# ruotianluo/ImageCaptioning.pytorch

Measured on NVIDIA H100. Metric: captions/sec at beam=5 seq_len=20, higher is better.
Workload: dtype f32 (fp32-grade: split-fp16 x3 tensor-core passes, fp32 accumulate)

## Files before the change

imagecaptioning.pytorch_b200/csrc/gemm_tc.cu:

```cuda
#include <cstdlib>

#include "common.cuh"
#include "ptx.cuh"

namespace capb200 {

namespace {

constexpr int BM = 128;
constexpr int BK = 64;
constexpr int kConsumers = 2;
constexpr int kThreads = 128 * (1 + kConsumers);

struct TcParams {
    CUtensorMap a_hi[kMaxSeg];
    CUtensorMap a_lo[kMaxSeg];
    CUtensorMap w_hi[kMaxSeg];
    CUtensorMap w_lo[kMaxSeg];
    int kblocks[kMaxSeg];
    int nseg;
    int M, N;
    float* C;
    long ldc;
    __half* C_hi;
    __half* C_lo;
    long ldcs;
    const float* bias;
    const float* row_bias;
    long ld_row_bias;
    int rows_per_group;
    int relu;
    const float* residual;
    long ld_res;
    int tiles_m, tiles_n;
    int lstm, H;
    const float* c_prev;
    long ld_cprev;
    const int* src_row;
    float* c_out;
    long ld_cout;
    const float* gather_bias;
    long ld_gb;
    const int* gather_idx;
    float* h_f;
    __half* h_hi;
    __half* h_lo;
    long ld_h;
    unsigned long long* trace;
};

__device__ __forceinline__ unsigned long long gtimer() {
    unsigned long long t;
    asm volatile("mov.u64 %0, %%globaltimer;" : "=l"(t));
    return t;
}
#define CAPB_TRACE(slot) do { if (TRACE && p.trace != nullptr) p.trace[(long)blockIdx.x * 16 + (slot)] = gtimer(); } while (0)

template <int BN, int PASSES>
struct TcCfg {
    static constexpr int kPlanes = (PASSES == 3) ? 2 : 1;
    static constexpr uint32_t kABytes = BM * BK * 2;
    static constexpr uint32_t kWBytes = BN * BK * 2;
    static constexpr uint32_t kStageBytes = kPlanes * (kABytes + kWBytes);
    static constexpr uint32_t kRingBudget = 227 * 1024 - 1024  - 256 ;
    static constexpr int kStages = kRingBudget / kStageBytes >= 8 ? 8 : kRingBudget / kStageBytes;
    static constexpr uint32_t kSmemBytes = kStages * kStageBytes + 1024  + 256 ;
    static_assert(BN == 64 || BN == 128 || BN == 160, "wgmma wrappers exist for N = 64, 128 and 160");
    static_assert(kWBytes % 1024 == 0, "operand tiles must keep the 1024-byte swizzle-atom alignment");
    static_assert(kStages >= 2, "need at least a double buffer");
    static_assert(kSmemBytes <= 227 * 1024, "shared memory of one H100 block");
};

template <int BN>
__device__ __forceinline__ void wgmma_f16(float* acc, uint64_t da, uint64_t db, int scale_d) {
    if (BN == 160) ptx::wgmma_f16_n160(acc, da, db, scale_d);
    else if (BN == 128) ptx::wgmma_f16_n128(acc, da, db, scale_d);
    else ptx::wgmma_f16_n64(acc, da, db, scale_d);
}

enum EpiKind : int {
    kEpiStore = 0,
    kEpiPlanes = 1,
    kEpiLstm = 2,
};

template <int BN>
__device__ __forceinline__ void epi_adds(const TcParams& p, float* acc, int r0, int c0) {
    const int ncol = p.N - c0;
    const int lim[2] = {r0 < p.M ? ncol : 0, r0 + 8 < p.M ? ncol : 0};
    if (p.bias != nullptr) {
        const float* b = p.bias + c0;
#pragma unroll
        for (int j = 0; j < BN / 8; ++j) {
#pragma unroll
            for (int e = 0; e < 2; ++e) {
                if (8 * j + e < ncol) {
                    const float x = __ldg(b + 8 * j + e);
                    acc[4 * j + e] += x;
                    acc[4 * j + 2 + e] += x;
                }
            }
        }
    }
    const float* tab[3][2];
#pragma unroll
    for (int h = 0; h < 2; ++h) {
        const int row = lim[h] > 0 ? r0 + 8 * h : 0;
        tab[0][h] = p.row_bias != nullptr ? p.row_bias + (long)(row / p.rows_per_group) * p.ld_row_bias + c0 : nullptr;
        tab[1][h] = p.gather_bias != nullptr ? p.gather_bias + (long)(lim[h] > 0 ? p.gather_idx[row] : 0) * p.ld_gb + c0 : nullptr;
        tab[2][h] = p.residual != nullptr ? p.residual + (long)row * p.ld_res + c0 : nullptr;
    }
#pragma unroll 1
    for (int t = 0; t < 3; ++t) {
        const float* const t0 = t == 0 ? tab[0][0] : t == 1 ? tab[1][0] : tab[2][0];
        const float* const t1 = t == 0 ? tab[0][1] : t == 1 ? tab[1][1] : tab[2][1];
        if (t0 == nullptr) continue;
#pragma unroll
        for (int j = 0; j < BN / 8; ++j) {
#pragma unroll
            for (int e = 0; e < 4; ++e) {
                const int k = 8 * j + (e & 1);
                if (k < lim[e >> 1]) acc[4 * j + e] += (e >> 1 ? t1 : t0)[k];
            }
        }
    }
    if (p.relu) {
#pragma unroll
        for (int i = 0; i < BN / 2; ++i) acc[i] = fmaxf(acc[i], 0.0f);
    }
}

template <int BN, bool TRACE>
__device__ __forceinline__ void epi_lstm(const TcParams& p, float* acc, int r0, int c0, int lane, int slot) {
    constexpr int kRuns = BN / 32;
    const bool odd = lane & 1;
    const bool upper = lane & 2;
    const int row = r0 + (odd ? 8 : 0);
    const int u0 = ((c0 - 2 * (lane & 3)) >> 2) + (upper ? 4 : 0);
    const bool row_ok = row < p.M;
    const bool full = u0 + 8 * (kRuns - 1) + 4 <= p.H;
    int src = row;
    if (p.src_row != nullptr && row_ok) src = p.src_row[row];
    const float* cprev = (row_ok && src >= 0 && p.c_prev != nullptr) ? p.c_prev + (long)src * p.ld_cprev + u0 : nullptr;
    float cp[BN / 8];
    if (cprev != nullptr && full && (reinterpret_cast<uintptr_t>(cprev) & 15) == 0) {
#pragma unroll
        for (int k = 0; k < kRuns; ++k) {
            const float4 v = *reinterpret_cast<const float4*>(cprev + 8 * k);
            cp[4 * k] = v.x; cp[4 * k + 1] = v.y; cp[4 * k + 2] = v.z; cp[4 * k + 3] = v.w;
        }
    } else {
#pragma unroll
        for (int i = 0; i < BN / 8; ++i) {
            const int du = 8 * (i / 4) + i % 4;
            cp[i] = (cprev != nullptr && u0 + du < p.H) ? cprev[du] : 0.0f;
        }
    }
    if (TRACE && slot >= 0) {
        float s = 0.0f;
#pragma unroll
        for (int i = 0; i < BN / 8; ++i) s += cp[i];
        asm volatile("" ::"f"(s));
        CAPB_TRACE(slot);
    }
    __syncwarp();
#pragma unroll
    for (int j = 0; j < BN / 8; ++j) {
        float* v = acc + 4 * j;
        const float s0 = __shfl_xor_sync(0xffffffffu, odd ? v[0] : v[2], 1);
        const float s1 = __shfl_xor_sync(0xffffffffu, odd ? v[1] : v[3], 1);
        const float gi = odd ? s0 : v[0], gf = odd ? s1 : v[1], gg = odd ? v[2] : s0, go = odd ? v[3] : s1;
        v[0] = gi; v[1] = gf; v[2] = gg; v[3] = go;
    }
#pragma unroll
    for (int k = 0; k < kRuns; ++k) {
#pragma unroll
        for (int t = 0; t < 2; ++t) {
            float* x = acc + 4 * (4 * k + t);
            float* y = acc + 4 * (4 * k + 2 + t);
#pragma unroll
            for (int g = 0; g < 4; ++g) {
                const float keep = upper ? y[g] : x[g];
                const float recv = __shfl_xor_sync(0xffffffffu, upper ? x[g] : y[g], 2);
                x[g] = upper ? recv : keep;
                y[g] = upper ? keep : recv;
            }
        }
    }
    float cn[BN / 8], hn[BN / 8];
#pragma unroll
    for (int i = 0; i < BN / 8; ++i) {
        const int k = i / 4, o = i % 4;
        const float* g = acc + 4 * (4 * k + (o >> 1) + 2 * (o & 1));
        cn[i] = fast_sigmoid(g[1]) * cp[i] + fast_sigmoid(g[0]) * fast_tanh(g[2]);
        hn[i] = fast_sigmoid(g[3]) * fast_tanh(cn[i]);
    }
    if (TRACE && slot >= 0) {
        float s = 0.0f;
#pragma unroll
        for (int i = 0; i < BN / 8; ++i) s += hn[i];
        asm volatile("" ::"f"(s));
        CAPB_TRACE(slot + 1);
    }
    if (row_ok) {
        float* const c_out = p.c_out + (long)row * p.ld_cout + u0;
        float* const h_f = p.h_f + (long)row * p.ld_h + u0;
        __half* const h_hi = p.h_hi + (long)row * p.ld_h + u0;
        __half* const h_lo = p.h_lo + (long)row * p.ld_h + u0;
        const bool planes = p.h_hi != nullptr;
        const uintptr_t a16 = reinterpret_cast<uintptr_t>(c_out) | reinterpret_cast<uintptr_t>(h_f);
        const uintptr_t a8 = planes ? reinterpret_cast<uintptr_t>(h_hi) | reinterpret_cast<uintptr_t>(h_lo) : 0;
        if (full && (a16 & 15) == 0 && (a8 & 7) == 0) {
#pragma unroll
            for (int k = 0; k < kRuns; ++k) {
                const float* c = cn + 4 * k;
                const float* h = hn + 4 * k;
                *reinterpret_cast<float4*>(c_out + 8 * k) = make_float4(c[0], c[1], c[2], c[3]);
                *reinterpret_cast<float4*>(h_f + 8 * k) = make_float4(h[0], h[1], h[2], h[3]);
                if (planes) {
                    __half hh[4], hl[4];
#pragma unroll
                    for (int o = 0; o < 4; ++o) split_f32(h[o], hh[o], hl[o]);
                    const __half2 hi01 = __halves2half2(hh[0], hh[1]), hi23 = __halves2half2(hh[2], hh[3]);
                    const __half2 lo01 = __halves2half2(hl[0], hl[1]), lo23 = __halves2half2(hl[2], hl[3]);
                    *reinterpret_cast<uint2*>(h_hi + 8 * k) = make_uint2(*reinterpret_cast<const uint32_t*>(&hi01), *reinterpret_cast<const uint32_t*>(&hi23));
                    *reinterpret_cast<uint2*>(h_lo + 8 * k) = make_uint2(*reinterpret_cast<const uint32_t*>(&lo01), *reinterpret_cast<const uint32_t*>(&lo23));
                }
            }
        } else {
#pragma unroll
            for (int i = 0; i < BN / 8; ++i) {
                const int du = 8 * (i / 4) + i % 4;
                if (u0 + du < p.H) {
                    c_out[du] = cn[i];
                    h_f[du] = hn[i];
                    if (planes) {
                        __half hh, hl;
                        split_f32(hn[i], hh, hl);
                        h_hi[du] = hh;
                        h_lo[du] = hl;
                    }
                }
            }
        }
    }
    if (TRACE && slot >= 0) CAPB_TRACE(slot + 2);
}

template <int BN, bool PLANES>
__device__ __forceinline__ void epi_store(const TcParams& p, const float* acc, int r0, int c0) {
    const int ncol = p.N - c0;
#pragma unroll
    for (int h = 0; h < 2; ++h) {
        const int row = r0 + 8 * h;
        if (row >= p.M) continue;
        if (p.C != nullptr) {
            float* const dst = p.C + (long)row * p.ldc + c0;
            if (ncol >= BN && (reinterpret_cast<uintptr_t>(dst) & 7) == 0) {
#pragma unroll
                for (int j = 0; j < BN / 8; ++j) *reinterpret_cast<float2*>(dst + 8 * j) = make_float2(acc[4 * j + 2 * h], acc[4 * j + 2 * h + 1]);
            } else {
#pragma unroll
                for (int j = 0; j < BN / 8; ++j) {
                    if (8 * j < ncol) dst[8 * j] = acc[4 * j + 2 * h];
                    if (8 * j + 1 < ncol) dst[8 * j + 1] = acc[4 * j + 2 * h + 1];
                }
            }
        }
        if (PLANES) {
            __half* const dh = p.C_hi + (long)row * p.ldcs + c0;
            __half* const dl = p.C_lo + (long)row * p.ldcs + c0;
            if (ncol >= BN && ((reinterpret_cast<uintptr_t>(dh) | reinterpret_cast<uintptr_t>(dl)) & 3) == 0) {
#pragma unroll
                for (int j = 0; j < BN / 8; ++j) {
                    __half h0, l0, h1, l1;
                    split_f32(acc[4 * j + 2 * h], h0, l0);
                    split_f32(acc[4 * j + 2 * h + 1], h1, l1);
                    *reinterpret_cast<__half2*>(dh + 8 * j) = __halves2half2(h0, h1);
                    *reinterpret_cast<__half2*>(dl + 8 * j) = __halves2half2(l0, l1);
                }
            } else {
#pragma unroll
                for (int j = 0; j < BN / 8; ++j) {
#pragma unroll
                    for (int e = 0; e < 2; ++e) {
                        __half hi, lo;
                        split_f32(acc[4 * j + 2 * h + e], hi, lo);
                        if (8 * j + e < ncol) { dh[8 * j + e] = hi; dl[8 * j + e] = lo; }
                    }
                }
            }
        }
    }
}

template <int BN, int EPI, bool TRACE>
__device__ __forceinline__ void epilogue_tile(const TcParams& p, float* acc, int m0, int n0, int tid, int slot) {
    const int warp = tid >> 5, lane = tid & 31;
    const int r0 = m0 + warp * 16 + (lane >> 2);
    const int c0 = n0 + 2 * (lane & 3);
    epi_adds<BN>(p, acc, r0, c0);
    if (EPI == kEpiLstm) epi_lstm<BN, TRACE>(p, acc, r0, c0, lane, slot);
    else epi_store<BN, EPI == kEpiPlanes>(p, acc, r0, c0);
}

template <int BN, int PASSES, int EPI, bool TRACE = false>
__global__ void __launch_bounds__(kThreads, 1) gemm_tc_kernel(const __grid_constant__ TcParams p) {
    using Cfg = TcCfg<BN, PASSES>;
    extern __shared__ uint8_t smem_raw[];
    uint8_t* smem = reinterpret_cast<uint8_t*>((reinterpret_cast<uintptr_t>(smem_raw) + 1023) & ~uintptr_t(1023));
    uint64_t* full_bar = reinterpret_cast<uint64_t*>(smem + Cfg::kStages * Cfg::kStageBytes);
    uint64_t* empty_bar = full_bar + Cfg::kStages;
    uint64_t* turn_bar = empty_bar + Cfg::kStages;

    const int wg = threadIdx.x >> 7;
    const int n_tiles = p.tiles_m * p.tiles_n;

    if (threadIdx.x == 0) {
        for (int s = 0; s < p.nseg; ++s) {
            ptx::prefetch_tmap(&p.a_hi[s]);
            ptx::prefetch_tmap(&p.w_hi[s]);
            if (PASSES == 3) {
                ptx::prefetch_tmap(&p.a_lo[s]);
                ptx::prefetch_tmap(&p.w_lo[s]);
            }
        }
        for (int i = 0; i < Cfg::kStages; ++i) {
            ptx::mbar_init(&full_bar[i], 1);
            ptx::mbar_init(&empty_bar[i], 1);
        }
        for (int c = 0; c < kConsumers; ++c) ptx::mbar_init(&turn_bar[c], 1);
        ptx::fence_mbar_init();
    }
    __syncthreads();
    if (threadIdx.x == 0) CAPB_TRACE(0);

    if (wg == 0) {
        ptx::setmaxnreg_dec<40>();
        if (threadIdx.x == 0) {
            int stage = 0;
            uint32_t phase = 0;
            for (int t = blockIdx.x; t < n_tiles; t += gridDim.x) {
                const int m0 = (t % p.tiles_m) * BM;
                const int n0 = (t / p.tiles_m) * BN;
                for (int s = 0; s < p.nseg; ++s) {
                    for (int kb = 0; kb < p.kblocks[s]; ++kb) {
                        ptx::mbar_wait(&empty_bar[stage], phase ^ 1);
                        uint8_t* st = smem + stage * Cfg::kStageBytes;
                        uint8_t* a_hi = st;
                        uint8_t* a_lo = st + Cfg::kABytes;
                        uint8_t* w_hi = st + Cfg::kABytes * Cfg::kPlanes;
                        uint8_t* w_lo = st + Cfg::kABytes * 2 + Cfg::kWBytes;
                        ptx::mbar_arrive_expect_tx(&full_bar[stage], Cfg::kStageBytes);
                        ptx::tma_load_2d(a_hi, &p.a_hi[s], &full_bar[stage], kb * BK, m0);
                        ptx::tma_load_2d(w_hi, &p.w_hi[s], &full_bar[stage], kb * BK, n0);
                        if (PASSES == 3) {
                            ptx::tma_load_2d(a_lo, &p.a_lo[s], &full_bar[stage], kb * BK, m0);
                            ptx::tma_load_2d(w_lo, &p.w_lo[s], &full_bar[stage], kb * BK, n0);
                        }
                        if (++stage == Cfg::kStages) { stage = 0; phase ^= 1; }
                    }
                }
            }
        }
    } else {
        ptx::setmaxnreg_inc<232>();
        const int cw = wg - 1;
        const int tid = threadIdx.x & 127;
        constexpr uint32_t kHalf = 64 * 128;
        int kb_tile = 0;
        for (int s = 0; s < p.nseg; ++s) kb_tile += p.kblocks[s];
        int mine = 0;
        for (int it = cw, t = blockIdx.x + cw * gridDim.x; t < n_tiles; it += 2, t += 2 * gridDim.x, ++mine) {
            const int m0 = (t % p.tiles_m) * BM;
            const int n0 = (t / p.tiles_m) * BN;
            if (it > 0) ptx::mbar_wait(&turn_bar[cw], (cw == 1 ? mine : mine - 1) & 1);
            if (TRACE && it == 1 && tid == 0) CAPB_TRACE(4);
            const long g0 = (long)it * kb_tile;
            int stage = (int)(g0 % Cfg::kStages);
            uint32_t phase = (uint32_t)(g0 / Cfg::kStages) & 1;
            float acc0[BN / 2], acc1[BN / 2];
#pragma unroll
            for (int i = 0; i < BN / 2; ++i) { acc0[i] = 0.0f; acc1[i] = 0.0f; }
            for (int s = 0; s < p.nseg; ++s) {
                for (int kb = 0; kb < p.kblocks[s]; ++kb) {
                    ptx::mbar_wait(&full_bar[stage], phase);
                    if (TRACE && it == 0 && s == 0 && kb == 0 && tid == 0) CAPB_TRACE(1);
                    const uint32_t st = ptx::smem_u32(smem + stage * Cfg::kStageBytes);
                    const uint32_t a_hi = st;
                    const uint32_t a_lo = st + Cfg::kABytes;
                    const uint32_t w_hi = st + Cfg::kABytes * Cfg::kPlanes;
                    const uint32_t w_lo = st + Cfg::kABytes * 2 + Cfg::kWBytes;
#pragma unroll
                    for (int i = 0; i < BN / 2; ++i) { ptx::reg_fence(acc0[i]); ptx::reg_fence(acc1[i]); }
                    ptx::wgmma_fence();
#pragma unroll
                    for (int k = 0; k < BK / 16; ++k) {
                        const uint32_t koff = k * 32;
                        const uint64_t dwh = ptx::make_smem_desc_sw128(w_hi + koff);
                        if (PASSES == 3) {
                            const uint64_t dwl = ptx::make_smem_desc_sw128(w_lo + koff);
                            wgmma_f16<BN>(acc0, ptx::make_smem_desc_sw128(a_hi + koff), dwl, 1);
                            wgmma_f16<BN>(acc1, ptx::make_smem_desc_sw128(a_hi + kHalf + koff), dwl, 1);
                            wgmma_f16<BN>(acc0, ptx::make_smem_desc_sw128(a_lo + koff), dwh, 1);
                            wgmma_f16<BN>(acc1, ptx::make_smem_desc_sw128(a_lo + kHalf + koff), dwh, 1);
                            wgmma_f16<BN>(acc0, ptx::make_smem_desc_sw128(a_hi + koff), dwh, 1);
                            wgmma_f16<BN>(acc1, ptx::make_smem_desc_sw128(a_hi + kHalf + koff), dwh, 1);
                        } else {
                            wgmma_f16<BN>(acc0, ptx::make_smem_desc_sw128(a_hi + koff), dwh, 1);
                            wgmma_f16<BN>(acc1, ptx::make_smem_desc_sw128(a_hi + kHalf + koff), dwh, 1);
                        }
                    }
                    ptx::wgmma_commit();
                    ptx::wgmma_wait<0>();
#pragma unroll
                    for (int i = 0; i < BN / 2; ++i) { ptx::reg_fence(acc0[i]); ptx::reg_fence(acc1[i]); }
                    if (tid == 0) ptx::mbar_arrive(&empty_bar[stage]);
                    if (++stage == Cfg::kStages) { stage = 0; phase ^= 1; }
                }
            }
            if (tid == 0) ptx::mbar_arrive(&turn_bar[cw ^ 1]);
            if (TRACE && it < 2 && tid == 0) CAPB_TRACE(2 + it);
#pragma unroll 1
            for (int h = 0; h < 2; ++h) {
                const int slot = (TRACE && it < 2 && h == 0 && tid == 0) ? 9 + 3 * it : -1;
                epilogue_tile<BN, EPI, TRACE>(p, acc0, m0 + 64 * h, n0, tid, slot);
#pragma unroll
                for (int i = 0; i < BN / 2; ++i) acc0[i] = acc1[i];
            }
            if (TRACE && it < 2 && tid == 0) CAPB_TRACE(6 + it);
        }
    }
    __syncthreads();
    if (threadIdx.x == 0) CAPB_TRACE(8);
}

typedef CUresult (*EncodeTiledFn)(CUtensorMap*, CUtensorMapDataType, cuuint32_t, void*, const cuuint64_t*, const cuuint64_t*,
                                  const cuuint32_t*, const cuuint32_t*, CUtensorMapInterleave, CUtensorMapSwizzle,
                                  CUtensorMapL2promotion, CUtensorMapFloatOOBfill);

EncodeTiledFn get_encode_fn() {
    static EncodeTiledFn fn = nullptr;
    if (fn == nullptr) {
        void* sym = nullptr;
        cudaDriverEntryPointQueryResult qres;
        if (cudaGetDriverEntryPoint("cuTensorMapEncodeTiled", &sym, cudaEnableDefault, &qres) != cudaSuccess || sym == nullptr) {
            return nullptr;
        }
        fn = reinterpret_cast<EncodeTiledFn>(sym);
    }
    return fn;
}

bool encode_plane(CUtensorMap* map, const __half* base, long rows, long K, long pitch, int box_rows, std::string* err) {
    EncodeTiledFn fn = get_encode_fn();
    if (fn == nullptr) { *err = "cuTensorMapEncodeTiled entry point not available"; return false; }
    cuuint64_t gdim[2] = {static_cast<cuuint64_t>(K), static_cast<cuuint64_t>(rows)};
    cuuint64_t gstride[1] = {static_cast<cuuint64_t>(pitch) * 2};
    cuuint32_t box[2] = {static_cast<cuuint32_t>(BK), static_cast<cuuint32_t>(box_rows)};
    cuuint32_t estr[2] = {1, 1};
    CUresult r = fn(map, CU_TENSOR_MAP_DATA_TYPE_FLOAT16, 2, const_cast<__half*>(base), gdim, gstride, box, estr,
                    CU_TENSOR_MAP_INTERLEAVE_NONE, CU_TENSOR_MAP_SWIZZLE_128B, CU_TENSOR_MAP_L2_PROMOTION_L2_256B,
                    CU_TENSOR_MAP_FLOAT_OOB_FILL_NONE);
    if (r != CUDA_SUCCESS) { *err = "cuTensorMapEncodeTiled failed with CUresult " + std::to_string((int)r); return false; }
    return true;
}

template <int BN, int PASSES, int EPI, bool TRACE = false>
int launch_cfg(const TcParams& prm, cudaStream_t stream) {
    using Cfg = TcCfg<BN, PASSES>;
    static std::atomic<unsigned long long> attr_set{0};
    if (first_use_on_device(attr_set)) {
        CAPB_CHECK_CUDA(cudaFuncSetAttribute(gemm_tc_kernel<BN, PASSES, EPI, TRACE>, cudaFuncAttributeMaxDynamicSharedMemorySize, Cfg::kSmemBytes));
    }
    TcParams prm2 = prm;
    prm2.tiles_n = cdiv(prm.N, BN);
    prm2.tiles_m = cdiv(prm.M, BM);
    const int n_tiles = prm2.tiles_n * prm2.tiles_m;
    const int sms = sm_count();
    gemm_tc_kernel<BN, PASSES, EPI, TRACE><<<n_tiles < sms ? n_tiles : sms, kThreads, Cfg::kSmemBytes, stream>>>(prm2);
    CAPB_CHECK_CUDA(cudaGetLastError());
    return 0;
}

template <int EPI>
int launch_kind(int bn, int passes, const TcParams& prm, cudaStream_t stream) {
    if (prm.trace != nullptr) {
        if (bn == 160) return launch_cfg<160, 3, EPI, true>(prm, stream);
        return bn == 128 ? launch_cfg<128, 3, EPI, true>(prm, stream) : launch_cfg<64, 3, EPI, true>(prm, stream);
    }
    if (bn == 160) return passes == 3 ? launch_cfg<160, 3, EPI>(prm, stream) : launch_cfg<160, 1, EPI>(prm, stream);
    if (bn == 128) return passes == 3 ? launch_cfg<128, 3, EPI>(prm, stream) : launch_cfg<128, 1, EPI>(prm, stream);
    return passes == 3 ? launch_cfg<64, 3, EPI>(prm, stream) : launch_cfg<64, 1, EPI>(prm, stream);
}

}

struct GemmTcPlan {
    TcParams prm;
    int passes;
    int bn;
};

static void fill_epilogue(TcParams& t, const GemmEpilogue& e) {
    t.C = e.C; t.ldc = e.ldc;
    t.C_hi = e.C_hi; t.C_lo = e.C_lo; t.ldcs = e.ldcs;
    t.bias = e.bias; t.row_bias = e.row_bias; t.ld_row_bias = e.ld_row_bias;
    t.rows_per_group = e.rows_per_group < 1 ? 1 : e.rows_per_group;
    t.relu = e.relu;
    t.residual = e.residual; t.ld_res = e.ld_res;
    t.lstm = e.lstm; t.H = e.H;
    t.c_prev = e.c_prev; t.ld_cprev = e.ld_cprev; t.src_row = e.src_row;
    t.c_out = e.c_out; t.ld_cout = e.ld_cout;
    t.gather_bias = e.gather_bias; t.ld_gb = e.ld_gb; t.gather_idx = e.gather_idx;
    t.h_f = e.h_f; t.h_hi = e.h_hi; t.h_lo = e.h_lo; t.ld_h = e.ld_h;
    t.trace = e.trace;
}

bool gemm_tc_supported(const GemmProblem& p, std::string* why) {
    auto bad = [&](const char* m) { if (why) *why = m; return false; };
    if (p.nseg < 1 || p.nseg > kMaxSeg) return bad("1..3 K-segments");
    for (int s = 0; s < p.nseg; ++s) {
        const GemmSeg& g = p.seg[s];
        if (g.A_hi == nullptr || g.W_hi == nullptr) return bad("split planes missing");
        if ((g.lda_h & 7) || (g.ldw_h & 7)) return bad("plane pitch must be a multiple of 8 elements (16 bytes)");
        if ((reinterpret_cast<uintptr_t>(g.A_hi) & 15) || (reinterpret_cast<uintptr_t>(g.W_hi) & 15)) return bad("plane base must be 16-byte aligned");
        if (g.K < 1) return bad("empty K-segment");
    }
    return true;
}

int gemm_tc_tile_n(int M, int N) {
    const int sms = sm_count();
    const int tiles_m = cdiv(M, BM);
    if (tiles_m * cdiv(N, 128) < sms / 2 && N > 64) return 64;
    const long cost128 = (long)cdiv(tiles_m * cdiv(N, 128), sms) * 128;
    const long cost160 = (long)cdiv(tiles_m * cdiv(N, 160), sms) * 160;
    return cost160 < cost128 ? 160 : 128;
}

GemmTcPlan* gemm_tc_plan_create(const GemmProblem& p, int passes) {
    std::string why;
    if (!gemm_tc_supported(p, &why)) { set_error("gemm_tc: unsupported problem: " + why); return nullptr; }
    if (passes != 1 && passes != 3) { set_error("gemm_tc: passes must be 1 or 3"); return nullptr; }
    GemmTcPlan* plan = new GemmTcPlan();
    memset(&plan->prm, 0, sizeof(TcParams));
    plan->passes = passes;
    plan->bn = gemm_tc_tile_n(p.M, p.N);
    TcParams& t = plan->prm;
    t.nseg = p.nseg;
    t.M = p.M;
    t.N = p.N;
    std::string err;
    for (int s = 0; s < p.nseg; ++s) {
        const GemmSeg& g = p.seg[s];
        t.kblocks[s] = cdiv(g.K, BK);
        bool ok = encode_plane(&t.a_hi[s], g.A_hi, p.M, g.K, g.lda_h, BM, &err) &&
                  encode_plane(&t.w_hi[s], g.W_hi, p.N, g.K, g.ldw_h, plan->bn, &err);
        if (ok && passes == 3) {
            if (g.A_lo == nullptr || g.W_lo == nullptr) { err = "lo planes missing for 3-pass mode"; ok = false; }
            ok = ok && encode_plane(&t.a_lo[s], g.A_lo, p.M, g.K, g.lda_h, BM, &err) &&
                 encode_plane(&t.w_lo[s], g.W_lo, p.N, g.K, g.ldw_h, plan->bn, &err);
        }
        if (!ok) { set_error("gemm_tc: " + err); delete plan; return nullptr; }
    }
    fill_epilogue(t, p.epi);
    return plan;
}

void gemm_tc_plan_destroy(GemmTcPlan* plan) { delete plan; }

int gemm_tc_plan_launch(GemmTcPlan* plan, const GemmEpilogue* epi_override, int M_override, cudaStream_t stream) {
    TcParams prm = plan->prm;
    if (epi_override != nullptr) fill_epilogue(prm, *epi_override);
    if (M_override > 0) {
        if (M_override > prm.M) { set_error("gemm_tc: M override exceeds the planned row count"); return 1; }
        prm.M = M_override;
    }
    if (prm.lstm && (prm.N != 4 * prm.H || prm.c_out == nullptr || prm.h_f == nullptr)) {
        set_error("gemm_tc: fused LSTM epilogue needs N == 4H, c_out and h_f");
        return 1;
    }
    if (prm.M <= 0 || prm.N <= 0) return 0;
    const int kind = prm.lstm ? kEpiLstm : prm.C_hi != nullptr ? kEpiPlanes : kEpiStore;
    if (prm.trace != nullptr && plan->passes != 3) { set_error("gemm_tc: the traced kernel is the 3-pass one"); return 1; }
    if (kind == kEpiLstm) return launch_kind<kEpiLstm>(plan->bn, plan->passes, prm, stream);
    if (kind == kEpiPlanes) return launch_kind<kEpiPlanes>(plan->bn, plan->passes, prm, stream);
    return launch_kind<kEpiStore>(plan->bn, plan->passes, prm, stream);
}

}
```

imagecaptioning.pytorch_b200/csrc/ptx.cuh:

```cuda
#pragma once
#include <cstdint>
#include <cuda.h>
#include <cuda_runtime.h>

namespace capb200 {
namespace ptx {

__device__ __forceinline__ uint32_t smem_u32(const void* p) {
    return static_cast<uint32_t>(__cvta_generic_to_shared(p));
}

__device__ __forceinline__ uint32_t elect_one() {
    uint32_t pred = 0;
    asm volatile(
        "{\n\t"
        ".reg .pred P;\n\t"
        "elect.sync _|P, 0xffffffff;\n\t"
        "selp.b32 %0, 1, 0, P;\n\t"
        "}\n"
        : "=r"(pred));
    return pred;
}

__device__ __forceinline__ void mbar_init(uint64_t* bar, uint32_t count) {
    asm volatile("mbarrier.init.shared::cta.b64 [%0], %1;" ::"r"(smem_u32(bar)), "r"(count) : "memory");
}
__device__ __forceinline__ void fence_mbar_init() {
    asm volatile("fence.mbarrier_init.release.cluster;" ::: "memory");
}
__device__ __forceinline__ void fence_proxy_async_smem() {
    asm volatile("fence.proxy.async.shared::cta;" ::: "memory");
}
__device__ __forceinline__ void mbar_arrive_expect_tx(uint64_t* bar, uint32_t bytes) {
    asm volatile("mbarrier.arrive.expect_tx.shared::cta.b64 _, [%0], %1;" ::"r"(smem_u32(bar)), "r"(bytes) : "memory");
}
__device__ __forceinline__ void mbar_arrive(uint64_t* bar) {
    asm volatile("mbarrier.arrive.shared::cta.b64 _, [%0];" ::"r"(smem_u32(bar)) : "memory");
}
__device__ __forceinline__ bool mbar_try_wait(uint64_t* bar, uint32_t parity) {
    uint32_t ok;
    asm volatile(
        "{\n\t"
        ".reg .pred P;\n\t"
        "mbarrier.try_wait.parity.shared::cta.b64 P, [%1], %2;\n\t"
        "selp.b32 %0, 1, 0, P;\n\t"
        "}\n"
        : "=r"(ok)
        : "r"(smem_u32(bar)), "r"(parity)
        : "memory");
    return ok != 0;
}
__device__ __forceinline__ void mbar_wait(uint64_t* bar, uint32_t parity) {
    uint32_t spins = 0;
    while (!mbar_try_wait(bar, parity)) {
        if (++spins > 200000000u) { __trap(); }
    }
}

template <int N>
__device__ __forceinline__ void setmaxnreg_dec() { asm volatile("setmaxnreg.dec.sync.aligned.u32 %0;" ::"n"(N)); }
template <int N>
__device__ __forceinline__ void setmaxnreg_inc() { asm volatile("setmaxnreg.inc.sync.aligned.u32 %0;" ::"n"(N)); }

__device__ __forceinline__ void prefetch_tmap(const CUtensorMap* m) {
    asm volatile("prefetch.tensormap [%0];" ::"l"(reinterpret_cast<uint64_t>(m)) : "memory");
}
__device__ __forceinline__ void tma_load_2d(void* smem_dst, const CUtensorMap* m, uint64_t* bar, int32_t c_inner, int32_t c_outer) {
    asm volatile(
        "cp.async.bulk.tensor.2d.shared::cluster.global.mbarrier::complete_tx::bytes [%0], [%1, {%3, %4}], [%2];"
        ::"r"(smem_u32(smem_dst)), "l"(reinterpret_cast<uint64_t>(m)), "r"(smem_u32(bar)), "r"(c_inner), "r"(c_outer)
        : "memory");
}

__device__ __forceinline__ void bulk_load_1d(void* smem_dst, const void* gsrc, uint32_t bytes, uint64_t* bar) {
    asm volatile("cp.async.bulk.shared::cluster.global.mbarrier::complete_tx::bytes [%0], [%1], %2, [%3];"
                 ::"r"(smem_u32(smem_dst)), "l"(reinterpret_cast<uint64_t>(gsrc)), "r"(bytes), "r"(smem_u32(bar)) : "memory");
}

__device__ __forceinline__ uint32_t cluster_ctaid_x() { uint32_t v; asm volatile("mov.u32 %0, %%cluster_ctaid.x;" : "=r"(v)); return v; }
__device__ __forceinline__ uint32_t cluster_ctaid_y() { uint32_t v; asm volatile("mov.u32 %0, %%cluster_ctaid.y;" : "=r"(v)); return v; }
__device__ __forceinline__ uint32_t cluster_ctarank() { uint32_t v; asm volatile("mov.u32 %0, %%cluster_ctarank;" : "=r"(v)); return v; }
__device__ __forceinline__ void cluster_sync_all() {
    asm volatile("barrier.cluster.arrive.release.aligned;" ::: "memory");
    asm volatile("barrier.cluster.wait.acquire.aligned;" ::: "memory");
}

__device__ __forceinline__ void wgmma_fence() { asm volatile("wgmma.fence.sync.aligned;" ::: "memory"); }
__device__ __forceinline__ void wgmma_commit() { asm volatile("wgmma.commit_group.sync.aligned;" ::: "memory"); }
template <int N>
__device__ __forceinline__ void wgmma_wait() { asm volatile("wgmma.wait_group.sync.aligned %0;" ::"n"(N) : "memory"); }
__device__ __forceinline__ void reg_fence(float& r) { asm volatile("" : "+f"(r)::"memory"); }

__device__ __forceinline__ uint64_t make_smem_desc_sw128(uint32_t smem_addr) {
    uint64_t d = 0;
    d |= static_cast<uint64_t>((smem_addr & 0x3FFFFu) >> 4);
    d |= static_cast<uint64_t>(1) << 16;
    d |= static_cast<uint64_t>(1024u >> 4) << 32;
    d |= static_cast<uint64_t>(1) << 62;
    return d;
}

__device__ __forceinline__ void wgmma_f16_n32(float* d, uint64_t desc_a, uint64_t desc_b, int scale_d) {
    asm volatile(
        "{\n\t.reg .pred p;\n\tsetp.ne.b32 p, %18, 0;\n\t"
        "wgmma.mma_async.sync.aligned.m64n32k16.f32.f16.f16 "
        "{"
        "%0, %1, %2, %3, %4, %5, %6, %7, %8, %9, %10, %11, %12, %13, %14, %15"
        "}, %16, %17, p, 1, 1, 0, 0;\n\t}\n"
        : "+f"(d[0]), "+f"(d[1]), "+f"(d[2]), "+f"(d[3]), "+f"(d[4]), "+f"(d[5]), "+f"(d[6]), "+f"(d[7]),
          "+f"(d[8]), "+f"(d[9]), "+f"(d[10]), "+f"(d[11]), "+f"(d[12]), "+f"(d[13]), "+f"(d[14]), "+f"(d[15])
        : "l"(desc_a), "l"(desc_b), "r"(scale_d));
}
__device__ __forceinline__ void wgmma_f16_n64(float* d, uint64_t desc_a, uint64_t desc_b, int scale_d) {
    asm volatile(
        "{\n\t.reg .pred p;\n\tsetp.ne.b32 p, %34, 0;\n\t"
        "wgmma.mma_async.sync.aligned.m64n64k16.f32.f16.f16 "
        "{"
        "%0, %1, %2, %3, %4, %5, %6, %7, %8, %9, %10, %11, %12, %13, %14, %15, "
        "%16, %17, %18, %19, %20, %21, %22, %23, %24, %25, %26, %27, %28, %29, %30, %31"
        "}, %32, %33, p, 1, 1, 0, 0;\n\t}\n"
        : "+f"(d[0]), "+f"(d[1]), "+f"(d[2]), "+f"(d[3]), "+f"(d[4]), "+f"(d[5]), "+f"(d[6]), "+f"(d[7]),
          "+f"(d[8]), "+f"(d[9]), "+f"(d[10]), "+f"(d[11]), "+f"(d[12]), "+f"(d[13]), "+f"(d[14]), "+f"(d[15]),
          "+f"(d[16]), "+f"(d[17]), "+f"(d[18]), "+f"(d[19]), "+f"(d[20]), "+f"(d[21]), "+f"(d[22]), "+f"(d[23]),
          "+f"(d[24]), "+f"(d[25]), "+f"(d[26]), "+f"(d[27]), "+f"(d[28]), "+f"(d[29]), "+f"(d[30]), "+f"(d[31])
        : "l"(desc_a), "l"(desc_b), "r"(scale_d));
}
__device__ __forceinline__ void wgmma_f16_n128(float* d, uint64_t desc_a, uint64_t desc_b, int scale_d) {
    asm volatile(
        "{\n\t.reg .pred p;\n\tsetp.ne.b32 p, %66, 0;\n\t"
        "wgmma.mma_async.sync.aligned.m64n128k16.f32.f16.f16 "
        "{"
        "%0, %1, %2, %3, %4, %5, %6, %7, %8, %9, %10, %11, %12, %13, %14, %15, "
        "%16, %17, %18, %19, %20, %21, %22, %23, %24, %25, %26, %27, %28, %29, %30, %31, "
        "%32, %33, %34, %35, %36, %37, %38, %39, %40, %41, %42, %43, %44, %45, %46, %47, "
        "%48, %49, %50, %51, %52, %53, %54, %55, %56, %57, %58, %59, %60, %61, %62, %63"
        "}, %64, %65, p, 1, 1, 0, 0;\n\t}\n"
        : "+f"(d[0]), "+f"(d[1]), "+f"(d[2]), "+f"(d[3]), "+f"(d[4]), "+f"(d[5]), "+f"(d[6]), "+f"(d[7]),
          "+f"(d[8]), "+f"(d[9]), "+f"(d[10]), "+f"(d[11]), "+f"(d[12]), "+f"(d[13]), "+f"(d[14]), "+f"(d[15]),
          "+f"(d[16]), "+f"(d[17]), "+f"(d[18]), "+f"(d[19]), "+f"(d[20]), "+f"(d[21]), "+f"(d[22]), "+f"(d[23]),
          "+f"(d[24]), "+f"(d[25]), "+f"(d[26]), "+f"(d[27]), "+f"(d[28]), "+f"(d[29]), "+f"(d[30]), "+f"(d[31]),
          "+f"(d[32]), "+f"(d[33]), "+f"(d[34]), "+f"(d[35]), "+f"(d[36]), "+f"(d[37]), "+f"(d[38]), "+f"(d[39]),
          "+f"(d[40]), "+f"(d[41]), "+f"(d[42]), "+f"(d[43]), "+f"(d[44]), "+f"(d[45]), "+f"(d[46]), "+f"(d[47]),
          "+f"(d[48]), "+f"(d[49]), "+f"(d[50]), "+f"(d[51]), "+f"(d[52]), "+f"(d[53]), "+f"(d[54]), "+f"(d[55]),
          "+f"(d[56]), "+f"(d[57]), "+f"(d[58]), "+f"(d[59]), "+f"(d[60]), "+f"(d[61]), "+f"(d[62]), "+f"(d[63])
        : "l"(desc_a), "l"(desc_b), "r"(scale_d));
}
__device__ __forceinline__ void wgmma_f16_n160(float* d, uint64_t desc_a, uint64_t desc_b, int scale_d) {
    asm volatile(
        "{\n\t.reg .pred p;\n\tsetp.ne.b32 p, %82, 0;\n\t"
        "wgmma.mma_async.sync.aligned.m64n160k16.f32.f16.f16 "
        "{"
        "%0, %1, %2, %3, %4, %5, %6, %7, %8, %9, %10, %11, %12, %13, %14, %15, "
        "%16, %17, %18, %19, %20, %21, %22, %23, %24, %25, %26, %27, %28, %29, %30, %31, "
        "%32, %33, %34, %35, %36, %37, %38, %39, %40, %41, %42, %43, %44, %45, %46, %47, "
        "%48, %49, %50, %51, %52, %53, %54, %55, %56, %57, %58, %59, %60, %61, %62, %63, "
        "%64, %65, %66, %67, %68, %69, %70, %71, %72, %73, %74, %75, %76, %77, %78, %79"
        "}, %80, %81, p, 1, 1, 0, 0;\n\t}\n"
        : "+f"(d[0]), "+f"(d[1]), "+f"(d[2]), "+f"(d[3]), "+f"(d[4]), "+f"(d[5]), "+f"(d[6]), "+f"(d[7]),
          "+f"(d[8]), "+f"(d[9]), "+f"(d[10]), "+f"(d[11]), "+f"(d[12]), "+f"(d[13]), "+f"(d[14]), "+f"(d[15]),
          "+f"(d[16]), "+f"(d[17]), "+f"(d[18]), "+f"(d[19]), "+f"(d[20]), "+f"(d[21]), "+f"(d[22]), "+f"(d[23]),
          "+f"(d[24]), "+f"(d[25]), "+f"(d[26]), "+f"(d[27]), "+f"(d[28]), "+f"(d[29]), "+f"(d[30]), "+f"(d[31]),
          "+f"(d[32]), "+f"(d[33]), "+f"(d[34]), "+f"(d[35]), "+f"(d[36]), "+f"(d[37]), "+f"(d[38]), "+f"(d[39]),
          "+f"(d[40]), "+f"(d[41]), "+f"(d[42]), "+f"(d[43]), "+f"(d[44]), "+f"(d[45]), "+f"(d[46]), "+f"(d[47]),
          "+f"(d[48]), "+f"(d[49]), "+f"(d[50]), "+f"(d[51]), "+f"(d[52]), "+f"(d[53]), "+f"(d[54]), "+f"(d[55]),
          "+f"(d[56]), "+f"(d[57]), "+f"(d[58]), "+f"(d[59]), "+f"(d[60]), "+f"(d[61]), "+f"(d[62]), "+f"(d[63]),
          "+f"(d[64]), "+f"(d[65]), "+f"(d[66]), "+f"(d[67]), "+f"(d[68]), "+f"(d[69]), "+f"(d[70]), "+f"(d[71]),
          "+f"(d[72]), "+f"(d[73]), "+f"(d[74]), "+f"(d[75]), "+f"(d[76]), "+f"(d[77]), "+f"(d[78]), "+f"(d[79])
        : "l"(desc_a), "l"(desc_b), "r"(scale_d));
}
__device__ __forceinline__ void wgmma_tf32_n32(float* d, uint64_t desc_a, uint64_t desc_b, int scale_d) {
    asm volatile(
        "{\n\t.reg .pred p;\n\tsetp.ne.b32 p, %18, 0;\n\t"
        "wgmma.mma_async.sync.aligned.m64n32k8.f32.tf32.tf32 "
        "{"
        "%0, %1, %2, %3, %4, %5, %6, %7, %8, %9, %10, %11, %12, %13, %14, %15"
        "}, %16, %17, p, 1, 1;\n\t}\n"
        : "+f"(d[0]), "+f"(d[1]), "+f"(d[2]), "+f"(d[3]), "+f"(d[4]), "+f"(d[5]), "+f"(d[6]), "+f"(d[7]),
          "+f"(d[8]), "+f"(d[9]), "+f"(d[10]), "+f"(d[11]), "+f"(d[12]), "+f"(d[13]), "+f"(d[14]), "+f"(d[15])
        : "l"(desc_a), "l"(desc_b), "r"(scale_d));
}
__device__ __forceinline__ void wgmma_tf32_n64(float* d, uint64_t desc_a, uint64_t desc_b, int scale_d) {
    asm volatile(
        "{\n\t.reg .pred p;\n\tsetp.ne.b32 p, %34, 0;\n\t"
        "wgmma.mma_async.sync.aligned.m64n64k8.f32.tf32.tf32 "
        "{"
        "%0, %1, %2, %3, %4, %5, %6, %7, %8, %9, %10, %11, %12, %13, %14, %15, "
        "%16, %17, %18, %19, %20, %21, %22, %23, %24, %25, %26, %27, %28, %29, %30, %31"
        "}, %32, %33, p, 1, 1;\n\t}\n"
        : "+f"(d[0]), "+f"(d[1]), "+f"(d[2]), "+f"(d[3]), "+f"(d[4]), "+f"(d[5]), "+f"(d[6]), "+f"(d[7]),
          "+f"(d[8]), "+f"(d[9]), "+f"(d[10]), "+f"(d[11]), "+f"(d[12]), "+f"(d[13]), "+f"(d[14]), "+f"(d[15]),
          "+f"(d[16]), "+f"(d[17]), "+f"(d[18]), "+f"(d[19]), "+f"(d[20]), "+f"(d[21]), "+f"(d[22]), "+f"(d[23]),
          "+f"(d[24]), "+f"(d[25]), "+f"(d[26]), "+f"(d[27]), "+f"(d[28]), "+f"(d[29]), "+f"(d[30]), "+f"(d[31])
        : "l"(desc_a), "l"(desc_b), "r"(scale_d));
}
__device__ __forceinline__ void wgmma_tf32_n128(float* d, uint64_t desc_a, uint64_t desc_b, int scale_d) {
    asm volatile(
        "{\n\t.reg .pred p;\n\tsetp.ne.b32 p, %66, 0;\n\t"
        "wgmma.mma_async.sync.aligned.m64n128k8.f32.tf32.tf32 "
        "{"
        "%0, %1, %2, %3, %4, %5, %6, %7, %8, %9, %10, %11, %12, %13, %14, %15, "
        "%16, %17, %18, %19, %20, %21, %22, %23, %24, %25, %26, %27, %28, %29, %30, %31, "
        "%32, %33, %34, %35, %36, %37, %38, %39, %40, %41, %42, %43, %44, %45, %46, %47, "
        "%48, %49, %50, %51, %52, %53, %54, %55, %56, %57, %58, %59, %60, %61, %62, %63"
        "}, %64, %65, p, 1, 1;\n\t}\n"
        : "+f"(d[0]), "+f"(d[1]), "+f"(d[2]), "+f"(d[3]), "+f"(d[4]), "+f"(d[5]), "+f"(d[6]), "+f"(d[7]),
          "+f"(d[8]), "+f"(d[9]), "+f"(d[10]), "+f"(d[11]), "+f"(d[12]), "+f"(d[13]), "+f"(d[14]), "+f"(d[15]),
          "+f"(d[16]), "+f"(d[17]), "+f"(d[18]), "+f"(d[19]), "+f"(d[20]), "+f"(d[21]), "+f"(d[22]), "+f"(d[23]),
          "+f"(d[24]), "+f"(d[25]), "+f"(d[26]), "+f"(d[27]), "+f"(d[28]), "+f"(d[29]), "+f"(d[30]), "+f"(d[31]),
          "+f"(d[32]), "+f"(d[33]), "+f"(d[34]), "+f"(d[35]), "+f"(d[36]), "+f"(d[37]), "+f"(d[38]), "+f"(d[39]),
          "+f"(d[40]), "+f"(d[41]), "+f"(d[42]), "+f"(d[43]), "+f"(d[44]), "+f"(d[45]), "+f"(d[46]), "+f"(d[47]),
          "+f"(d[48]), "+f"(d[49]), "+f"(d[50]), "+f"(d[51]), "+f"(d[52]), "+f"(d[53]), "+f"(d[54]), "+f"(d[55]),
          "+f"(d[56]), "+f"(d[57]), "+f"(d[58]), "+f"(d[59]), "+f"(d[60]), "+f"(d[61]), "+f"(d[62]), "+f"(d[63])
        : "l"(desc_a), "l"(desc_b), "r"(scale_d));
}

}
}
```

Baseline: 22790.

## Keep one wgmma group in flight with BK=32 stages for wide GEMMs

Adds a non-draining consumer schedule in which each consumer warpgroup waits with wgmma_wait<1> instead of draining after every k-block. The stage ring buffer is released one step late, and the turn barrier is handed to the other consumer early, on the last k-block. This schedule uses BK=32 with 64-byte swizzle, which gives more and smaller stages. A host heuristic or environment variable picks it when there are more tiles than SMs and tiles_n >= tiles_m; the LSTM epilogue always keeps the old draining path. It aims to overlap tensor-core work with barrier and TMA latency, at the cost of smaller k-blocks that add per-stage overhead, and it encodes two sets of tensor maps per plan.

Result: slower. 22430 (median of 6 runs) (-1.5%).

```diff
diff --git a/imagecaptioning.pytorch_b200/csrc/gemm_tc.cu b/imagecaptioning.pytorch_b200/csrc/gemm_tc.cu
--- a/imagecaptioning.pytorch_b200/csrc/gemm_tc.cu
+++ b/imagecaptioning.pytorch_b200/csrc/gemm_tc.cu
@@ -8,7 +8,8 @@
 namespace {
 
 constexpr int BM = 128;
-constexpr int BK = 64;
+template <bool DRAIN>
+constexpr int kBK = DRAIN ? 64 : 32;
 constexpr int kConsumers = 2;
 constexpr int kThreads = 128 * (1 + kConsumers);
 
@@ -56,20 +57,29 @@
 }
 #define CAPB_TRACE(slot) do { if (TRACE && p.trace != nullptr) p.trace[(long)blockIdx.x * 16 + (slot)] = gtimer(); } while (0)
 
-template <int BN, int PASSES>
+template <int BN, int PASSES, int BK>
 struct TcCfg {
     static constexpr int kPlanes = (PASSES == 3) ? 2 : 1;
-    static constexpr uint32_t kABytes = BM * BK * 2;
-    static constexpr uint32_t kWBytes = BN * BK * 2;
+    static constexpr uint32_t kRowBytes = BK * 2;
+    static constexpr uint32_t kAtomBytes = 8 * kRowBytes;
+    static constexpr uint32_t kABytes = BM * kRowBytes;
+    static constexpr uint32_t kWBytes = BN * kRowBytes;
     static constexpr uint32_t kStageBytes = kPlanes * (kABytes + kWBytes);
     static constexpr uint32_t kRingBudget = 227 * 1024 - 1024  - 256 ;
     static constexpr int kStages = kRingBudget / kStageBytes >= 8 ? 8 : kRingBudget / kStageBytes;
     static constexpr uint32_t kSmemBytes = kStages * kStageBytes + 1024  + 256 ;
+    static_assert(BK == 32 || BK == 64, "64- or 128-byte swizzle rows");
     static_assert(BN == 64 || BN == 128 || BN == 160, "wgmma wrappers exist for N = 64, 128 and 160");
-    static_assert(kWBytes % 1024 == 0, "operand tiles must keep the 1024-byte swizzle-atom alignment");
-    static_assert(kStages >= 2, "need at least a double buffer");
+    static_assert(kABytes % kAtomBytes == 0 && kWBytes % kAtomBytes == 0 && (64 * kRowBytes) % kAtomBytes == 0,
+                  "operand tiles and the second m64 half of A must keep the swizzle-atom alignment");
+    static_assert(kStages >= (BK == 32 ? 4 : 2), "the in-flight schedule holds two stages per consumer; the draining one double-buffers");
     static_assert(kSmemBytes <= 227 * 1024, "shared memory of one H100 block");
 };
+
+template <int BK>
+__device__ __forceinline__ uint64_t smem_desc(uint32_t addr) {
+    return BK == 64 ? ptx::make_smem_desc_sw128(addr) : ptx::make_smem_desc_sw64(addr);
+}
 
 template <int BN>
 __device__ __forceinline__ void wgmma_f16(float* acc, uint64_t da, uint64_t db, int scale_d) {
@@ -304,9 +314,10 @@
     else epi_store<BN, EPI == kEpiPlanes>(p, acc, r0, c0);
 }
 
-template <int BN, int PASSES, int EPI, bool TRACE = false>
+template <int BN, int PASSES, int EPI, bool TRACE = false, bool DRAIN = false>
 __global__ void __launch_bounds__(kThreads, 1) gemm_tc_kernel(const __grid_constant__ TcParams p) {
-    using Cfg = TcCfg<BN, PASSES>;
+    constexpr int BK = kBK<DRAIN>;
+    using Cfg = TcCfg<BN, PASSES, BK>;
     extern __shared__ uint8_t smem_raw[];
     uint8_t* smem = reinterpret_cast<uint8_t*>((reinterpret_cast<uintptr_t>(smem_raw) + 1023) & ~uintptr_t(1023));
     uint64_t* full_bar = reinterpret_cast<uint64_t*>(smem + Cfg::kStages * Cfg::kStageBytes);
@@ -367,7 +378,7 @@
         ptx::setmaxnreg_inc<232>();
         const int cw = wg - 1;
         const int tid = threadIdx.x & 127;
-        constexpr uint32_t kHalf = 64 * 128;
+        constexpr uint32_t kHalf = 64 * Cfg::kRowBytes;
         int kb_tile = 0;
         for (int s = 0; s < p.nseg; ++s) kb_tile += p.kblocks[s];
         int mine = 0;
@@ -382,6 +393,8 @@
             float acc0[BN / 2], acc1[BN / 2];
 #pragma unroll
             for (int i = 0; i < BN / 2; ++i) { acc0[i] = 0.0f; acc1[i] = 0.0f; }
+            int left = kb_tile;
+            int in_flight = -1;
             for (int s = 0; s < p.nseg; ++s) {
                 for (int kb = 0; kb < p.kblocks[s]; ++kb) {
                     ptx::mbar_wait(&full_bar[stage], phase);
@@ -391,35 +404,51 @@
                     const uint32_t a_lo = st + Cfg::kABytes;
                     const uint32_t w_hi = st + Cfg::kABytes * Cfg::kPlanes;
                     const uint32_t w_lo = st + Cfg::kABytes * 2 + Cfg::kWBytes;
-#pragma unroll
-                    for (int i = 0; i < BN / 2; ++i) { ptx::reg_fence(acc0[i]); ptx::reg_fence(acc1[i]); }
+                    if (DRAIN) {
+#pragma unroll
+                        for (int i = 0; i < BN / 2; ++i) { ptx::reg_fence(acc0[i]); ptx::reg_fence(acc1[i]); }
+                    }
                     ptx::wgmma_fence();
 #pragma unroll
                     for (int k = 0; k < BK / 16; ++k) {
                         const uint32_t koff = k * 32;
-                        const uint64_t dwh = ptx::make_smem_desc_sw128(w_hi + koff);
+                        const uint64_t dwh = smem_desc<BK>(w_hi + koff);
                         if (PASSES == 3) {
-                            const uint64_t dwl = ptx::make_smem_desc_sw128(w_lo + koff);
-                            wgmma_f16<BN>(acc0, ptx::make_smem_desc_sw128(a_hi + koff), dwl, 1);
-                            wgmma_f16<BN>(acc1, ptx::make_smem_desc_sw128(a_hi + kHalf + koff), dwl, 1);
-                            wgmma_f16<BN>(acc0, ptx::make_smem_desc_sw128(a_lo + koff), dwh, 1);
-                            wgmma_f16<BN>(acc1, ptx::make_smem_desc_sw128(a_lo + kHalf + koff), dwh, 1);
-                            wgmma_f16<BN>(acc0, ptx::make_smem_desc_sw128(a_hi + koff), dwh, 1);
-                            wgmma_f16<BN>(acc1, ptx::make_smem_desc_sw128(a_hi + kHalf + koff), dwh, 1);
+                            const uint64_t dwl = smem_desc<BK>(w_lo + koff);
+                            wgmma_f16<BN>(acc0, smem_desc<BK>(a_hi + koff), dwl, 1);
+                            wgmma_f16<BN>(acc1, smem_desc<BK>(a_hi + kHalf + koff), dwl, 1);
+                            wgmma_f16<BN>(acc0, smem_desc<BK>(a_lo + koff), dwh, 1);
+                            wgmma_f16<BN>(acc1, smem_desc<BK>(a_lo + kHalf + koff), dwh, 1);
+                            wgmma_f16<BN>(acc0, smem_desc<BK>(a_hi + koff), dwh, 1);
+                            wgmma_f16<BN>(acc1, smem_desc<BK>(a_hi + kHalf + koff), dwh, 1);
                         } else {
-                            wgmma_f16<BN>(acc0, ptx::make_smem_desc_sw128(a_hi + koff), dwh, 1);
-                            wgmma_f16<BN>(acc1, ptx::make_smem_desc_sw128(a_hi + kHalf + koff), dwh, 1);
+                            wgmma_f16<BN>(acc0, smem_desc<BK>(a_hi + koff), dwh, 1);
+                            wgmma_f16<BN>(acc1, smem_desc<BK>(a_hi + kHalf + koff), dwh, 1);
                         }
                     }
                     ptx::wgmma_commit();
-                    ptx::wgmma_wait<0>();
-#pragma unroll
-                    for (int i = 0; i < BN / 2; ++i) { ptx::reg_fence(acc0[i]); ptx::reg_fence(acc1[i]); }
-                    if (tid == 0) ptx::mbar_arrive(&empty_bar[stage]);
+                    if (DRAIN) {
+                        ptx::wgmma_wait<0>();
+#pragma unroll
+                        for (int i = 0; i < BN / 2; ++i) { ptx::reg_fence(acc0[i]); ptx::reg_fence(acc1[i]); }
+                        if (tid == 0) ptx::mbar_arrive(&empty_bar[stage]);
+                    } else {
+                        ptx::mbar_arrive_if(&turn_bar[cw ^ 1], --left == 0 && tid == 0);
+                        ptx::wgmma_wait<1>();
+                        ptx::mbar_arrive_if(&empty_bar[in_flight < 0 ? 0 : in_flight], in_flight >= 0 && tid == 0);
+                        in_flight = stage;
+                    }
                     if (++stage == Cfg::kStages) { stage = 0; phase ^= 1; }
                 }
             }
-            if (tid == 0) ptx::mbar_arrive(&turn_bar[cw ^ 1]);
+            if (DRAIN) {
+                if (tid == 0) ptx::mbar_arrive(&turn_bar[cw ^ 1]);
+            } else {
+                ptx::wgmma_wait<0>();
+#pragma unroll
+                for (int i = 0; i < BN / 2; ++i) { ptx::reg_fence(acc0[i]); ptx::reg_fence(acc1[i]); }
+                if (tid == 0) ptx::mbar_arrive(&empty_bar[in_flight]);
+            }
             if (TRACE && it < 2 && tid == 0) CAPB_TRACE(2 + it);
 #pragma unroll 1
             for (int h = 0; h < 2; ++h) {
@@ -452,54 +481,62 @@
     return fn;
 }
 
-bool encode_plane(CUtensorMap* map, const __half* base, long rows, long K, long pitch, int box_rows, std::string* err) {
+bool encode_plane(CUtensorMap* map, const __half* base, long rows, long K, long pitch, int box_rows, int bk, std::string* err) {
     EncodeTiledFn fn = get_encode_fn();
     if (fn == nullptr) { *err = "cuTensorMapEncodeTiled entry point not available"; return false; }
     cuuint64_t gdim[2] = {static_cast<cuuint64_t>(K), static_cast<cuuint64_t>(rows)};
     cuuint64_t gstride[1] = {static_cast<cuuint64_t>(pitch) * 2};
-    cuuint32_t box[2] = {static_cast<cuuint32_t>(BK), static_cast<cuuint32_t>(box_rows)};
+    cuuint32_t box[2] = {static_cast<cuuint32_t>(bk), static_cast<cuuint32_t>(box_rows)};
     cuuint32_t estr[2] = {1, 1};
     CUresult r = fn(map, CU_TENSOR_MAP_DATA_TYPE_FLOAT16, 2, const_cast<__half*>(base), gdim, gstride, box, estr,
-                    CU_TENSOR_MAP_INTERLEAVE_NONE, CU_TENSOR_MAP_SWIZZLE_128B, CU_TENSOR_MAP_L2_PROMOTION_L2_256B,
-                    CU_TENSOR_MAP_FLOAT_OOB_FILL_NONE);
+                    CU_TENSOR_MAP_INTERLEAVE_NONE, bk == 64 ? CU_TENSOR_MAP_SWIZZLE_128B : CU_TENSOR_MAP_SWIZZLE_64B,
+                    CU_TENSOR_MAP_L2_PROMOTION_L2_256B, CU_TENSOR_MAP_FLOAT_OOB_FILL_NONE);
     if (r != CUDA_SUCCESS) { *err = "cuTensorMapEncodeTiled failed with CUresult " + std::to_string((int)r); return false; }
     return true;
 }
 
-template <int BN, int PASSES, int EPI, bool TRACE = false>
+template <int BN, int PASSES, int EPI, bool TRACE, bool DRAIN>
 int launch_cfg(const TcParams& prm, cudaStream_t stream) {
-    using Cfg = TcCfg<BN, PASSES>;
+    using Cfg = TcCfg<BN, PASSES, kBK<DRAIN>>;
     static std::atomic<unsigned long long> attr_set{0};
     if (first_use_on_device(attr_set)) {
-        CAPB_CHECK_CUDA(cudaFuncSetAttribute(gemm_tc_kernel<BN, PASSES, EPI, TRACE>, cudaFuncAttributeMaxDynamicSharedMemorySize, Cfg::kSmemBytes));
+        CAPB_CHECK_CUDA(cudaFuncSetAttribute(gemm_tc_kernel<BN, PASSES, EPI, TRACE, DRAIN>, cudaFuncAttributeMaxDynamicSharedMemorySize,
+                                             Cfg::kSmemBytes));
     }
     TcParams prm2 = prm;
     prm2.tiles_n = cdiv(prm.N, BN);
     prm2.tiles_m = cdiv(prm.M, BM);
     const int n_tiles = prm2.tiles_n * prm2.tiles_m;
     const int sms = sm_count();
-    gemm_tc_kernel<BN, PASSES, EPI, TRACE><<<n_tiles < sms ? n_tiles : sms, kThreads, Cfg::kSmemBytes, stream>>>(prm2);
+    gemm_tc_kernel<BN, PASSES, EPI, TRACE, DRAIN><<<n_tiles < sms ? n_tiles : sms, kThreads, Cfg::kSmemBytes, stream>>>(prm2);
     CAPB_CHECK_CUDA(cudaGetLastError());
     return 0;
 }
 
-template <int EPI>
+template <int EPI, bool DRAIN>
 int launch_kind(int bn, int passes, const TcParams& prm, cudaStream_t stream) {
     if (prm.trace != nullptr) {
-        if (bn == 160) return launch_cfg<160, 3, EPI, true>(prm, stream);
-        return bn == 128 ? launch_cfg<128, 3, EPI, true>(prm, stream) : launch_cfg<64, 3, EPI, true>(prm, stream);
-    }
-    if (bn == 160) return passes == 3 ? launch_cfg<160, 3, EPI>(prm, stream) : launch_cfg<160, 1, EPI>(prm, stream);
-    if (bn == 128) return passes == 3 ? launch_cfg<128, 3, EPI>(prm, stream) : launch_cfg<128, 1, EPI>(prm, stream);
-    return passes == 3 ? launch_cfg<64, 3, EPI>(prm, stream) : launch_cfg<64, 1, EPI>(prm, stream);
+        if (bn == 160) return launch_cfg<160, 3, EPI, true, DRAIN>(prm, stream);
+        return bn == 128 ? launch_cfg<128, 3, EPI, true, DRAIN>(prm, stream) : launch_cfg<64, 3, EPI, true, DRAIN>(prm, stream);
+    }
+    if (bn == 160) return passes == 3 ? launch_cfg<160, 3, EPI, false, DRAIN>(prm, stream) : launch_cfg<160, 1, EPI, false, DRAIN>(prm, stream);
+    if (bn == 128) return passes == 3 ? launch_cfg<128, 3, EPI, false, DRAIN>(prm, stream) : launch_cfg<128, 1, EPI, false, DRAIN>(prm, stream);
+    return passes == 3 ? launch_cfg<64, 3, EPI, false, DRAIN>(prm, stream) : launch_cfg<64, 1, EPI, false, DRAIN>(prm, stream);
+}
+
+template <int EPI>
+int launch_kind(bool drain, int bn, int passes, const TcParams& prm, cudaStream_t stream) {
+    return drain ? launch_kind<EPI, true>(bn, passes, prm, stream) : launch_kind<EPI, false>(bn, passes, prm, stream);
 }
 
 }
 
 struct GemmTcPlan {
-    TcParams prm;
+    TcParams prm[2];
+    GemmEpilogue epi;
     int passes;
     int bn;
+    bool drain;
 };
 
 static void fill_epilogue(TcParams& t, const GemmEpilogue& e) {
@@ -539,40 +576,54 @@
     return cost160 < cost128 ? 160 : 128;
 }
 
+static bool gemm_tc_inflight(int M, int N, int bn) {
+    const char* force = getenv("CAPB200_GEMM_SCHEDULE");
+    if (force != nullptr && strcmp(force, "drain") == 0) return false;
+    if (force != nullptr && strcmp(force, "inflight") == 0) return true;
+    const int tiles_m = cdiv(M, BM), tiles_n = cdiv(N, bn);
+    return tiles_m * tiles_n > sm_count() && tiles_n >= tiles_m;
+}
+
 GemmTcPlan* gemm_tc_plan_create(const GemmProblem& p, int passes) {
     std::string why;
     if (!gemm_tc_supported(p, &why)) { set_error("gemm_tc: unsupported problem: " + why); return nullptr; }
     if (passes != 1 && passes != 3) { set_error("gemm_tc: passes must be 1 or 3"); return nullptr; }
     GemmTcPlan* plan = new GemmTcPlan();
-    memset(&plan->prm, 0, sizeof(TcParams));
+    memset(plan->prm, 0, sizeof(plan->prm));
     plan->passes = passes;
     plan->bn = gemm_tc_tile_n(p.M, p.N);
-    TcParams& t = plan->prm;
-    t.nseg = p.nseg;
-    t.M = p.M;
-    t.N = p.N;
+    plan->drain = !gemm_tc_inflight(p.M, p.N, plan->bn);
     std::string err;
-    for (int s = 0; s < p.nseg; ++s) {
-        const GemmSeg& g = p.seg[s];
-        t.kblocks[s] = cdiv(g.K, BK);
-        bool ok = encode_plane(&t.a_hi[s], g.A_hi, p.M, g.K, g.lda_h, BM, &err) &&
-                  encode_plane(&t.w_hi[s], g.W_hi, p.N, g.K, g.ldw_h, plan->bn, &err);
-        if (ok && passes == 3) {
-            if (g.A_lo == nullptr || g.W_lo == nullptr) { err = "lo planes missing for 3-pass mode"; ok = false; }
-            ok = ok && encode_plane(&t.a_lo[s], g.A_lo, p.M, g.K, g.lda_h, BM, &err) &&
-                 encode_plane(&t.w_lo[s], g.W_lo, p.N, g.K, g.ldw_h, plan->bn, &err);
-        }
-        if (!ok) { set_error("gemm_tc: " + err); delete plan; return nullptr; }
-    }
-    fill_epilogue(t, p.epi);
+    for (int d = 0; d < 2; ++d) {
+        const int bk = d ? kBK<true> : kBK<false>;
+        TcParams& t = plan->prm[d];
+        t.nseg = p.nseg;
+        t.M = p.M;
+        t.N = p.N;
+        for (int s = 0; s < p.nseg; ++s) {
+            const GemmSeg& g = p.seg[s];
+            t.kblocks[s] = cdiv(g.K, bk);
+            bool ok = encode_plane(&t.a_hi[s], g.A_hi, p.M, g.K, g.lda_h, BM, bk, &err) &&
+                      encode_plane(&t.w_hi[s], g.W_hi, p.N, g.K, g.ldw_h, plan->bn, bk, &err);
+            if (ok && passes == 3) {
+                if (g.A_lo == nullptr || g.W_lo == nullptr) { err = "lo planes missing for 3-pass mode"; ok = false; }
+                ok = ok && encode_plane(&t.a_lo[s], g.A_lo, p.M, g.K, g.lda_h, BM, bk, &err) &&
+                     encode_plane(&t.w_lo[s], g.W_lo, p.N, g.K, g.ldw_h, plan->bn, bk, &err);
+            }
+            if (!ok) { set_error("gemm_tc: " + err); delete plan; return nullptr; }
+        }
+    }
+    plan->epi = p.epi;
     return plan;
 }
 
 void gemm_tc_plan_destroy(GemmTcPlan* plan) { delete plan; }
 
 int gemm_tc_plan_launch(GemmTcPlan* plan, const GemmEpilogue* epi_override, int M_override, cudaStream_t stream) {
-    TcParams prm = plan->prm;
-    if (epi_override != nullptr) fill_epilogue(prm, *epi_override);
+    const GemmEpilogue& e = epi_override != nullptr ? *epi_override : plan->epi;
+    const int kind = e.lstm ? kEpiLstm : e.C_hi != nullptr ? kEpiPlanes : kEpiStore;
+    TcParams prm = plan->prm[plan->drain || kind == kEpiLstm ? 1 : 0];
+    fill_epilogue(prm, e);
     if (M_override > 0) {
         if (M_override > prm.M) { set_error("gemm_tc: M override exceeds the planned row count"); return 1; }
         prm.M = M_override;
@@ -582,11 +633,10 @@
         return 1;
     }
     if (prm.M <= 0 || prm.N <= 0) return 0;
-    const int kind = prm.lstm ? kEpiLstm : prm.C_hi != nullptr ? kEpiPlanes : kEpiStore;
     if (prm.trace != nullptr && plan->passes != 3) { set_error("gemm_tc: the traced kernel is the 3-pass one"); return 1; }
-    if (kind == kEpiLstm) return launch_kind<kEpiLstm>(plan->bn, plan->passes, prm, stream);
-    if (kind == kEpiPlanes) return launch_kind<kEpiPlanes>(plan->bn, plan->passes, prm, stream);
-    return launch_kind<kEpiStore>(plan->bn, plan->passes, prm, stream);
-}
-
-}
+    if (kind == kEpiLstm) return launch_kind<kEpiLstm, true>(plan->bn, plan->passes, prm, stream);
+    if (kind == kEpiPlanes) return launch_kind<kEpiPlanes>(plan->drain, plan->bn, plan->passes, prm, stream);
+    return launch_kind<kEpiStore>(plan->drain, plan->bn, plan->passes, prm, stream);
+}
+
+}
diff --git a/imagecaptioning.pytorch_b200/csrc/ptx.cuh b/imagecaptioning.pytorch_b200/csrc/ptx.cuh
--- a/imagecaptioning.pytorch_b200/csrc/ptx.cuh
+++ b/imagecaptioning.pytorch_b200/csrc/ptx.cuh
@@ -36,6 +36,15 @@
 }
 __device__ __forceinline__ void mbar_arrive(uint64_t* bar) {
     asm volatile("mbarrier.arrive.shared::cta.b64 _, [%0];" ::"r"(smem_u32(bar)) : "memory");
+}
+__device__ __forceinline__ void mbar_arrive_if(uint64_t* bar, bool pred) {
+    asm volatile(
+        "{\n\t"
+        ".reg .pred P;\n\t"
+        "setp.ne.b32 P, %1, 0;\n\t"
+        "@P mbarrier.arrive.shared::cta.b64 _, [%0];\n\t"
+        "}\n"
+        ::"r"(smem_u32(bar)), "r"(static_cast<uint32_t>(pred)) : "memory");
 }
 __device__ __forceinline__ bool mbar_try_wait(uint64_t* bar, uint32_t parity) {
     uint32_t ok;
@@ -100,6 +109,15 @@
     return d;
 }
 
+__device__ __forceinline__ uint64_t make_smem_desc_sw64(uint32_t smem_addr) {
+    uint64_t d = 0;
+    d |= static_cast<uint64_t>((smem_addr & 0x3FFFFu) >> 4);
+    d |= static_cast<uint64_t>(1) << 16;
+    d |= static_cast<uint64_t>(512u >> 4) << 32;
+    d |= static_cast<uint64_t>(2) << 62;
+    return d;
+}
+
 __device__ __forceinline__ void wgmma_f16_n32(float* d, uint64_t desc_a, uint64_t desc_b, int scale_d) {
     asm volatile(
         "{\n\t.reg .pred p;\n\tsetp.ne.b32 p, %18, 0;\n\t"
```
